# UPM-ROB-Lab/Vision-basedSensor

Measured on AMD Instinct MI355X. Metric: frames/sec (track->3D) at 1280x1024, 169 markers, higher is better.
Workload: dtype u8+f64; 1 GPU; BASELINE config 3/4: 4096 synthetic 1280x1024 gray uint8 frames per GPU (13x13 dots, seeded jitter+noise), resident in HBM; fused track->3D table + last-seen displacement; frames_per_gpu=4096, internal_batch=1536, pass_streams=2, markers=169, channels=1, world_size=1, backend=none (single process), distinct_devices=1, tracked_observations=692224, xyz_solved=692224, ncc_ambiguous_pixels=205, ncc_exact_pixels=11244250, ncc_counter_frames=839680

## Files before the change

include/vbs.h:

```cpp
#ifndef VBS_H
#define VBS_H

#include <stdint.h>

#ifdef __cplusplus
extern "C" {
#endif

#define VBS_OK          0
#define VBS_EINVAL     -1
#define VBS_ECAPACITY  -2
#define VBS_EHIP       -3
#define VBS_ENOMEM     -4
#define VBS_EINTERNAL  -5

#define VBS_DET_COLS    6
#define VBS_TABLE_COLS 10
#define VBS_FLAG_TRACKED 1
#define VBS_FLAG_XYZ     2
#define VBS_DISP_COLS   5
#define VBS_PLANE_COLS  5
#define VBS_DEVPLANE_COLS 9

typedef struct vbs_handle vbs_handle;
// ... 3 lines not shown
    float dist[5];
    float R[9];
    float T[3];
    float marker_diameter_mm;
} vbs_camera;

int vbs_create(int device, int height, int width, int max_markers, int max_batch, vbs_handle** out);
int vbs_destroy(vbs_handle* h);
const char* vbs_last_error(const vbs_handle* h);
int vbs_version(void);
#define VBS_OPT_GRAY_COEFFS      1
#define VBS_OPT_FORCE_SEQ_MATCH  2
#define VBS_OPT_NCC_MARGIN       4
#define VBS_OPT_STAGE_IMPL       5
#define VBS_OPT_BLUR_IMPL        6
#define VBS_OPT_PASS_STREAMS     7
#define VBS_OPT_LATENCY_FRAMES   8
int vbs_set_option(vbs_handle* h, int option, int value);
int vbs_mjpeg_probe(const uint8_t* jpeg, int64_t size, int32_t* info);
int vbs_mjpeg_entropy_batch(const uint8_t* buf, const int64_t* offs, const int32_t* sizes, int n, const int32_t* info,
                            uint32_t* ent, uint32_t* tab, int64_t* frame_base, int64_t* regions, uint16_t* qt, int32_t* status,
                            int threads);
int vbs_mjpeg_reconstruct(const uint32_t* ent, const uint32_t* tab, const int64_t* frame_base, const uint16_t* qt, int n,
                          const int32_t* info, uint8_t* planes, uint8_t* out, int64_t out_frame, int64_t out_row, void* stream);
#define VBS_MJPEG_SCAN_ALIGN      16
#define VBS_MJPEG_SCAN_GUARD      16
#define VBS_MJPEG_HUFF_SET_BYTES  8928
#define VBS_MJPEG_SUBSEQ_BITS     1024
#define VBS_MJPEG_DEVICE_BITS_MAX 2147418112
#define VBS_MJPEG_SHORT           1
int vbs_mjpeg_scan_batch(const uint8_t* buf, int64_t buf_size, const int64_t* offs, const int64_t* sizes, int n, const int32_t* info,
                         uint8_t* stage, int64_t stage_cap, int64_t* scan_off, int64_t* scan_bits, int32_t* table_set, void* sets,
                         int32_t* n_sets, int64_t* regions, uint16_t* qt, int32_t* status, int threads);
int vbs_mjpeg_huffman_device(const uint8_t* stage, const int64_t* scan_off, const int64_t* scan_bits, const int32_t* table_set,
                             const void* sets, int n_sets, int n, const int32_t* info, int subseq_bits, uint32_t* ent, uint32_t* tab,
                             int64_t* frame_base, int32_t* status, void* stream);
#define VBS_JPEG_BLOCK_BITS_MAX 1660
#define VBS_JPEG_HEADER_BYTES   623
int vbs_jpeg_encode_workspace(int width, int height, int n, int64_t* workspace_bytes, int64_t* payload_bytes,
                              int64_t* frame_bound);
int vbs_jpeg_encode(const uint8_t* frames, int n, int width, int height, int64_t stride_n, int64_t stride_row, int quality,
                    void* workspace, int64_t workspace_bytes, uint8_t* payload, int64_t payload_bytes, int64_t* offsets,
                    int32_t* sizes, void* stream);
int vbs_draw_tracking(const uint8_t* frames, int n, int height, int width, int64_t stride_n, int64_t stride_row,
                      const double* det, int max_markers, const float* table, const double* ref_xy, int m_ref,
                      int32_t* lastw, uint8_t* out, void* stream);
int vbs_contour_lut(uint8_t out[256]);
int vbs_step_lut(uint32_t out[256]);
int64_t vbs_format_csv(const int64_t* frameno, const int64_t* row, const int64_t* col, const double* const* fcols, int nf,
                       int64_t n, char* buf, int64_t cap, int threads);
int vbs_gaussian_taps_q8(int ksize, double sigma, int32_t* out);
int vbs_ncc_template(int l, double sigma, double* g, double* stats);
int vbs_ncc_trim_guard(int l, double sigma, int height, int width, double tbar_shift, double* min_d0);

int vbs_set_undistort(vbs_handle* h, const double* K9, const double* dist, int ndist, double* newK9, void* stream);
int vbs_undistort_frames(vbs_handle* h, const uint8_t* frames, int n, int channels, int64_t stride_n,
                         int64_t stride_row, uint8_t* out, void* stream);

int vbs_bgr2gray(vbs_handle* h, const uint8_t* frames, int n, int64_t stride_n, int64_t stride_row, uint8_t* gray,
                 void* stream);

int vbs_find_markers(vbs_handle* h, const uint8_t* frames, int n, int channels, int64_t stride_n,
                     int64_t stride_row, uint8_t* mask, uint8_t* area_mask, void* stream);

int vbs_ncc_map(vbs_handle* h, const uint8_t* frames, int n, int channels, int64_t stride_n,
                int64_t stride_row, double* ncc, void* stream);
int vbs_normxcorr2(vbs_handle* h, const uint8_t* area_mask, int n, double* ncc, uint8_t* mask,
                   void* stream);
int vbs_normxcorr2_general(int device, const double* tmpl, int th, int tw, const double* image, int h, int w, int mode,
                           double* out, void* stream);
int vbs_profile(vbs_handle* h, int enable);
int vbs_profile_read(vbs_handle* h, char* buf, int cap);
int vbs_frame_stats(vbs_handle* h, uint32_t* out, int n);
int vbs_stage_tables(vbs_handle* h, int n, uint32_t* ncomp, uint64_t* band_sums, uint32_t* area_first, int64_t* area_sums,
                     uint16_t* probe, uint32_t* slow);
int vbs_ellipse_table(vbs_handle* h, int n, double* out);
int vbs_ncc_counters(vbs_handle* h, uint64_t out[3], int reset);

int vbs_undistort_points(int device, const double* pts, int n, const vbs_camera* cam, double* out,
                         void* stream);
int vbs_calculate_3d(int device, const double* uvd, int n, const vbs_camera* cam, double* xyz,
                     int32_t* ok, void* stream);

#define VBS_PNP_SAMPLE            6
#define VBS_PNP_MAX_POINTS     1024
#define VBS_PNP_MAX_HYPOTHESES 4096
#define VBS_PNP_FEW_POINTS        1
#define VBS_PNP_NO_HYPOTHESIS     2
int vbs_pnp_ransac(int device, const double* world, int n_points, const double* image, const float* table,
                   const uint8_t* valid, int n_problems, const vbs_camera* cam, const int32_t* samples, int n_hyp,
                   double reproj_px, int32_t* hyp_count, double* hyp_pose, int32_t* status, double* pose,
                   int32_t* inlier_count, uint8_t* inlier_mask, double* errors, int32_t* winner, void* stream);

#define VBS_CALIB_MAX_VIEWS   64
#define VBS_CALIB_FEW_VIEWS    1
#define VBS_CALIB_DEGENERATE   2
int vbs_calibrate_camera(int device, const double* obj, int n_points, const double* img, int n_views, const uint8_t* view_mask,
                         int n_problems, int w, int h, int max_iter, double* homography, int32_t* view_void, int32_t* status,
                         double* K4, double* dist, double* R, double* T, double* rms, double* view_rms, double* std_intrinsics,
                         int32_t* iterations, void* stream);

int vbs_marker_center(vbs_handle* h, const uint8_t* mask, const uint8_t* area_mask, int n,
                      double* det, int32_t* counts, void* stream);

#define VBS_DIAM_COLS        24
#define VBS_DIAM_STATS_COLS   5
// ... 204 lines not shown
```

vision-basedsensor_amd/_lib.py:

```python
import ctypes as C
import os

_HERE = os.path.dirname(os.path.abspath(__file__))
LIB_PATH = os.path.join(_HERE, "csrc", "libvbs.so")

VBS_OK, VBS_EINVAL, VBS_ECAPACITY, VBS_EHIP, VBS_ENOMEM, VBS_EINTERNAL = 0, -1, -2, -3, -4, -5
DET_COLS, TABLE_COLS, DISP_COLS, PLANE_COLS, DEVPLANE_COLS = 6, 10, 5, 5, 9
FLAG_TRACKED, FLAG_XYZ = 1, 2
JPEG_BLOCK_BITS_MAX, JPEG_HEADER_BYTES = 1660, 623
MJPEG_SCAN_ALIGN, MJPEG_SCAN_GUARD, MJPEG_HUFF_SET_BYTES, MJPEG_SUBSEQ_BITS, MJPEG_SHORT = 16, 16, 8928, 1024, 1
SERIES_CHUNK, SERIES_REC_COLS, STATS_COLS, WINDOW_COLS = 32, 5, 5, 4
FIR_MAX_TAPS, FIR_TILE, AXIS_COLS, TOTAL_COLS = 255, 64, 4, 5
STEP_MAX_WINDOW, STEP_MAX_STEPS = 64, 64
POSE_COLS, POSEFIELD_COLS, POSE_GROUP = 8, 6, 8
FIELD_FRAMES, FIELD_MAX_SLOTS, FIELD_MAX_POINTS, PATCH_COLS, PATCH_GROUP = 4, 1024, 65536, 8, 8
PROJ_SLOTS, PROJ_CHUNK, PROJ_ROWS, PROJ_WG_SLOTS, PROJ_MAX_ROWS, PROJ_MAX_FRAMES, PROJ_MAX_SLOTS = 4, 64, 64, 16, 8192, 1048576, 1024
FIT_GROUP, PEAK_COLS = 4, 7
ENV_TILE, ENV_MAX_HALF = 64, 127
KIN_TILE, KIN_MAX_HALF, KIN_MAX_DEGREE = 64, 127, 3
MOM_CHUNK, MOM_WG_SLOTS, MOM_MAX_SLOTS = 32, 16, 1024
MODES_MAX, MODES_MAX_DIM, MODES_SWEEPS, MODES_MAX_ITERS, SCORE_GROUP = 16, 3072, 10, 4096, 8
STRAIN_COLS, LSTRAIN_COLS, MOTION_GROUP, LSTRAIN_GROUP, STRAIN_MAX_NBR = 16, 8, 8, 8, 12
ROBUST_MAX_HALF, ROBUST_TILE = 31, 64
DIAM_COLS, DIAM_STATS_COLS, DIAM_MAX_EXTENT = 24, 5, 512
PNP_SAMPLE, PNP_MAX_POINTS, PNP_MAX_HYPOTHESES, PNP_FEW_POINTS, PNP_NO_HYPOTHESIS = 6, 1024, 4096, 1, 2
CHESS_MAX_CANDIDATES, CHESS_MAX_PATTERN, CHESS_MAX_WIN = 256, 256, 15
CALIB_MAX_VIEWS, CALIB_FEW_VIEWS, CALIB_DEGENERATE = 64, 1, 2
IDS_MAX_MARKERS, IDS_MAX_LAYERS = 1024, 16
RETRACK_MAX, RETRACK_STATE_COLS, RETRACK_INFO_COLS = 1024, 6, 4
UNCERT_CAM, UNCERT_COV_COLS, UNCERT_DCOV_COLS, UNCERT_TOTAL_COLS, UNCERT_GROUP = 16, 7, 8, 8, 4
UNCERT_REF_COLS, UNCERT_WORK_COLS, NOISE_COLS = 55, 61, 10
POSECOV_COLS, POSECOV_GROUP = 17, 4
OPT_GRAY_COEFFS, OPT_FORCE_SEQ_MATCH, OPT_NCC_MARGIN, OPT_STAGE_IMPL, OPT_BLUR_IMPL, OPT_PASS_STREAMS, OPT_LATENCY_FRAMES = 1, 2, 4, 5, 6, 7, 8

SYMBOLS = ("vbs_create", "vbs_destroy", "vbs_last_error", "vbs_version", "vbs_contour_lut",
           "vbs_gaussian_taps_q8", "vbs_ncc_template", "vbs_ncc_trim_guard", "vbs_set_undistort", "vbs_undistort_frames", "vbs_find_markers", "vbs_ncc_map", "vbs_normxcorr2",
           "vbs_profile", "vbs_profile_read", "vbs_frame_stats", "vbs_undistort_points", "vbs_calculate_3d", "vbs_marker_center",
           "vbs_track", "vbs_solve3d", "vbs_track_to_3d", "vbs_displacement", "vbs_displacement_range", "vbs_displacement_f64",
           "vbs_plane_fit", "vbs_assign_ids", "vbs_set_option", "vbs_bgr2gray", "vbs_ncc_counters", "vbs_normxcorr2_general",
           "vbs_stage_tables", "vbs_ellipse_table", "vbs_deviation_plane", "vbs_format_csv", "vbs_mjpeg_probe", "vbs_mjpeg_entropy_batch",
           "vbs_mjpeg_reconstruct", "vbs_jpeg_encode_workspace", "vbs_jpeg_encode", "vbs_draw_tracking",
           "vbs_series_chunks", "vbs_series_stats", "vbs_series_stats_f64", "vbs_series_partial", "vbs_series_merge",
           "vbs_window_means", "vbs_displacement_from_frame", "vbs_mjpeg_scan_batch", "vbs_mjpeg_huffman_device",
           "vbs_step_lut", "vbs_threshold_bits", "vbs_measure_markers", "vbs_pnp_ransac",
           "vbs_chess_workspace", "vbs_chess_corners", "vbs_corner_subpix", "vbs_calibrate_camera",
           "vbs_retrack_workspace", "vbs_retrack",
           "vbs_uncert_points", "vbs_uncert_cov", "vbs_uncert_total", "vbs_pixel_noise", "vbs_pose_cov",
           "vbs_axis_displacement", "vbs_fir_series_f64",
           "vbs_step_response_f64", "vbs_find_steps_f64", "vbs_dwell_stats_f64", "vbs_pose_series",
           "vbs_field_map_f64", "vbs_patch_stats_f64", "vbs_project_series_f64", "vbs_harmonic_fit_f64", "vbs_window_moments_f64", "vbs_window_fit_f64",
           "vbs_poly_moments_f64", "vbs_poly_fit_f64",
           "vbs_motion_series_f64", "vbs_local_strain_f64", "vbs_hampel_series_f64",
           "vbs_cross_moments_f64", "vbs_covariance_f64", "vbs_leading_modes_f64", "vbs_mode_scores_f64")


class Camera(C.Structure):
    _fields_ = [("K", C.c_float * 9), ("dist", C.c_float * 5), ("R", C.c_float * 9),
                ("T", C.c_float * 3), ("marker_diameter_mm", C.c_float)]


class VbsError(RuntimeError):
    pass


def status_text(status: int, max_markers: int = 0) -> str:
    if status == VBS_ECAPACITY:
        return ("the frame exceeds the device workspace (more than 30720 runs in a mask, more than "
                f"{max_markers or 'max_markers'} band components, more than about 512 contours, or a contour thousands of rows "
                "long whose vertex moments would leave 64 bits)")
    if status == VBS_EINTERNAL:
        return ("a kernel's internal hand-shake timed out: the frame's result is not to be trusted (bounded wait expired; "
                "see VBS_EINTERNAL in include/vbs.h)")
    return "unexpected device status"


_lib = None


def lib():
    global _lib
    if _lib is not None:
        return _lib
    if not os.path.exists(LIB_PATH):
        raise VbsError(f"{LIB_PATH} is missing: build it with `python -c 'import __graft_entry__ as g; "
                       f"g.build()'` (hipcc, gfx950). There is no CPU fallback.")
    try:
        import torch
    except ImportError:
        pass
    L = C.CDLL(LIB_PATH)
    vp, i32, i64, f64 = C.c_void_p, C.c_int, C.c_int64, C.c_double
    cam_p = C.POINTER(Camera)
    sig = {
        "vbs_create": (i32, [i32, i32, i32, i32, i32, C.POINTER(vp)]),
        "vbs_destroy": (i32, [vp]),
        "vbs_last_error": (C.c_char_p, [vp]),
        "vbs_version": (i32, []),
        "vbs_contour_lut": (i32, [vp]),
        "vbs_gaussian_taps_q8": (i32, [i32, f64, vp]),
        "vbs_ncc_template": (i32, [i32, f64, vp, vp]),
        "vbs_ncc_trim_guard": (i32, [i32, f64, i32, i32, f64, vp]),
        "vbs_set_undistort": (i32, [vp, vp, vp, i32, vp, vp]),
        "vbs_undistort_frames": (i32, [vp, vp, i32, i32, i64, i64, vp, vp]),
        "vbs_find_markers": (i32, [vp, vp, i32, i32, i64, i64, vp, vp, vp]),
        "vbs_ncc_map": (i32, [vp, vp, i32, i32, i64, i64, vp, vp]),
        "vbs_normxcorr2": (i32, [vp, vp, i32, vp, vp, vp]),
        "vbs_profile": (i32, [vp, i32]),
        "vbs_profile_read": (i32, [vp, vp, i32]),
        "vbs_frame_stats": (i32, [vp, vp, i32]),
        "vbs_undistort_points": (i32, [i32, vp, i32, cam_p, vp, vp]),
        "vbs_calculate_3d": (i32, [i32, vp, i32, cam_p, vp, vp, vp]),
        "vbs_marker_center": (i32, [vp, vp, vp, i32, vp, vp, vp]),
        "vbs_track": (i32, [vp, vp, vp, i32, vp, i32, f64, vp, vp]),
        "vbs_solve3d": (i32, [vp, vp, i32, i32, cam_p, f64, vp]),
        "vbs_track_to_3d": (i32, [vp, vp, i32, i32, i64, i64, vp, i32, f64, cam_p, f64, vp, vp, vp, vp]),
        "vbs_displacement": (i32, [vp, vp, i32, i32, i32, f64, f64, vp, vp]),
        "vbs_displacement_range": (i32, [vp, vp, i32, i32, i32, f64, f64, i32, i32, vp, vp]),
        "vbs_displacement_f64": (i32, [i32, vp, i32, i32, i32, f64, f64, vp, vp]),
        "vbs_plane_fit": (i32, [vp, vp, i32, i32, vp, vp]),
        "vbs_assign_ids": (i32, [vp, vp, vp, i32, i32, vp, vp, i32, vp, vp]),
        "vbs_set_option": (i32, [vp, i32, i32]),
        "vbs_bgr2gray": (i32, [vp, vp, i32, i64, i64, vp, vp]),
        "vbs_ncc_counters": (i32, [vp, vp, i32]),
        "vbs_normxcorr2_general": (i32, [i32, vp, i32, i32, vp, i32, i32, i32, vp, vp]),
        "vbs_stage_tables": (i32, [vp, i32, vp, vp, vp, vp, vp, vp]),
        "vbs_ellipse_table": (i32, [vp, i32, vp]),
        "vbs_deviation_plane": (i32, [vp, vp, vp, vp, vp, vp, i32, i32, f64, vp, vp, vp]),
        "vbs_format_csv": (i64, [vp, vp, vp, vp, i32, i64, vp, i64, i32]),
        "vbs_mjpeg_probe": (i32, [vp, i64, vp]),
        "vbs_mjpeg_entropy_batch": (i32, [vp, vp, vp, i32, vp, vp, vp, vp, vp, vp, vp, i32]),
        "vbs_mjpeg_reconstruct": (i32, [vp, vp, vp, vp, i32, vp, vp, vp, i64, i64, vp]),
        "vbs_mjpeg_scan_batch": (i32, [vp, i64, vp, vp, i32, vp, vp, i64, vp, vp, vp, vp, vp, vp, vp, vp, i32]),
        "vbs_mjpeg_huffman_device": (i32, [vp, vp, vp, vp, vp, i32, i32, vp, i32, vp, vp, vp, vp, vp]),
        "vbs_jpeg_encode_workspace": (i32, [i32, i32, i32, vp, vp, vp]),
        "vbs_jpeg_encode": (i32, [vp, i32, i32, i32, i64, i64, i32, vp, i64, vp, i64, vp, vp, vp]),
        "vbs_draw_tracking": (i32, [vp, i32, i32, i32, i64, i64, vp, i32, vp, vp, i32, vp, vp, vp]),
        "vbs_series_chunks": (i32, [i32, i32]),
        "vbs_series_stats": (i32, [vp, vp, i32, i32, i32, vp, vp, vp]),
        "vbs_series_stats_f64": (i32, [i32, vp, i32, i32, i32, vp, vp, vp, vp]),
        "vbs_series_partial": (i32, [vp, vp, i32, i32, i32, vp, vp]),
        "vbs_series_merge": (i32, [vp, vp, i32, i32, vp, vp, vp]),
        "vbs_window_means": (i32, [vp, vp, i32, i32, vp, i32, vp, vp]),
        "vbs_displacement_from_frame": (i32, [vp, vp, i32, i32, i32, vp, vp]),
        "vbs_axis_displacement": (i32, [vp, vp, i32, i32, i32, vp, i32, i32, vp, vp, vp]),
        "vbs_fir_series_f64": (i32, [i32, vp, i32, i32, i32, i32, vp, i32, f64, i32, i32, vp, vp]),
        "vbs_step_response_f64": (i32, [i32, vp, i32, i32, i32, i32, i32, i32, vp, vp]),
        "vbs_find_steps_f64": (i32, [i32, vp, i32, i32, i32, i32, f64, i32, vp, vp]),
        "vbs_dwell_stats_f64": (i32, [i32, vp, i32, i32, i32, i32, vp, i32, i32, i32, vp, vp]),
        "vbs_pose_series": (i32, [vp, vp, i32, i32, i32, vp, vp, vp, i32, f64, f64, i32, i32, vp, vp, vp, vp]),
        "vbs_field_map_f64": (i32, [i32, vp, i32, i32, i32, i32, vp, vp, i32, f64, i32, i32, vp, vp]),
        "vbs_patch_stats_f64": (i32, [i32, vp, i32, i32, i32, vp, i32, f64, f64, vp, vp]),
        "vbs_project_series_f64": (i32, [i32, vp, i32, i32, i32, i32, vp, i32, vp, vp]),
        "vbs_harmonic_fit_f64": (i32, [i32, vp, i32, i32, i32, i32, i32, f64, vp, vp, vp]),
        "vbs_window_moments_f64": (i32, [i32, vp, i32, i32, i32, i32, vp, vp, i32, i32, i32, vp, vp]),
# ... 47 lines not shown
```

vision-basedsensor_amd/csrc/k_stage.hip:

```cpp
#include "stage_common.h"

#define ST_NT_SMALL 256
#define ST_NT 768

struct StageGeom {
    int H, W, WW, G, NB, R, maxm;
    u32 off_rec, off_bot, off_pq, off_mb, off_tmp;
    u32 mrec_cap, mrec_stride;
    u32 rec_cap, pq_cap, mom_comps;
    int stop;
    int retry;
};

template <int NT>
__device__ __forceinline__ u32 st_scan(u32 v, u32* tmp, u32* total) {
    const int lane = threadIdx.x & 63, wave = threadIdx.x >> 6;
    u32 inc = v;
#pragma unroll
    for (int d = 1; d < 64; d <<= 1) {
        const u32 t = __shfl_up(inc, d);
        if (lane >= d) inc += t;
    }
    if (lane == 63) tmp[wave] = inc;
    __syncthreads();
    if (wave == 0) {
        const u32 t = lane < NT / 64 ? tmp[lane] : 0u;
        u32 ti = t;
#pragma unroll
        for (int d = 1; d < NT / 64; d <<= 1) {
            const u32 o = __shfl_up(ti, d);
            if (lane >= d) ti += o;
        }
        if (lane < NT / 64) tmp[lane] = ti - t;
        if (lane == NT / 64 - 1) tmp[16] = ti;
    }
    __syncthreads();
    const u32 ex = inc - v + tmp[wave];
    *total = tmp[16];
    __syncthreads();
    return ex;
}

template <int NT>
__device__ __forceinline__ u32 seg_resolve(unsigned short* P, u32 sbase, u32 nseg, const unsigned short* rec_sid,
                                           const u32* rec_pos, u32 nrec, const u32* seg_pos, u32* comp_pos,
                                           unsigned short* cidmap, u32* tmp, u32 limit, const PairQ& Q) {
    const int tid = threadIdx.x;
    {
        const int np = min(*Q.n, Q.cap);
        for (int i = tid; i < np; i += NT) { const u32 pr = Q.q[i]; ccl_union(P, pr >> 16, pr & 0xFFFFu); }
    }
    __syncthreads();
    for (u32 i = 0; i < nseg; ++i) {
        u32 x = sbase + i, p;
        while ((p = ((volatile unsigned short*)P)[x]) != x) x = p;
        if (x != sbase + i) P[sbase + i] = (unsigned short)x;
    }
    __syncthreads();
    u32 nroot = 0;
    for (u32 i = 0; i < nseg; ++i) nroot += (P[sbase + i] == sbase + i);
    u32 ncomp;
    u32 c0 = st_scan<NT>(nroot, tmp, &ncomp);
    if (ncomp > limit) return NONE32;
    for (u32 i = 0; i < nseg; ++i)
        if (P[sbase + i] == sbase + i) { comp_pos[c0] = NONE32; P[sbase + i] = (unsigned short)(0x8000u | c0++); }
    __syncthreads();
    for (u32 i = 0; i < nseg; ++i) {
        const u32 v = P[sbase + i];
        if (!(v & 0x8000u)) P[sbase + i] = (unsigned short)(P[v] & 0x7FFFu);
    }
    __syncthreads();
    if (seg_pos) { for (u32 i = 0; i < nseg; ++i) atomicMin(&comp_pos[P[sbase + i] & 0x7FFFu], seg_pos[sbase + i]); }
    else { for (u32 r = tid; r < nrec; r += NT) atomicMin(&comp_pos[P[rec_sid[r]] & 0x7FFFu], rec_pos[r]); }
    __syncthreads();
    for (u32 c = tid; c < ncomp; c += NT) {
        const u32 p = comp_pos[c];
        u32 rank = 0;
        for (u32 q = 0; q < ncomp; ++q) rank += comp_pos[q] < p;
        cidmap[c] = (unsigned short)rank;
    }
    __syncthreads();
    return ncomp;
}

template <int NS, int NT>
__global__ __launch_bounds__(NT, 3) void k_stage(const u64* __restrict__ mask_all, const u64* __restrict__ area_all,
                                                    u32* __restrict__ ncomp_all, u64* __restrict__ band_sums,
                                                    u32* __restrict__ area_first, i64* __restrict__ area_sums,
                                                    unsigned short* __restrict__ probe_all, u32* __restrict__ fstat,
                                                    u32* __restrict__ slow_flag, u32* __restrict__ slow_total,
                                                    u32* __restrict__ mrec_all, StageGeom geo) {
    extern __shared__ __align__(16) unsigned char smem[];
    unsigned short* P = reinterpret_cast<unsigned short*>(smem);
    unsigned char* recb = smem + geo.off_rec;
    unsigned char* botb = smem + geo.off_bot;
    PairQ Q;
    Q.q = reinterpret_cast<u32*>(smem + geo.off_pq);
    Q.cap = (int)geo.pq_cap;
    u32* mb_cnt = reinterpret_cast<u32*>(smem + geo.off_mb);
    u32* mb_req = mb_cnt + NT;
    u32* tmp = reinterpret_cast<u32*>(smem + geo.off_tmp);
    int* misc = reinterpret_cast<int*>(tmp + 32);
    const int n = blockIdx.x, tid = threadIdx.x, lane = tid & 63, wave = tid >> 6;
    const int H = geo.H, W = geo.W, WW = geo.WW, G = geo.G, R = geo.R, maxm = geo.maxm;
    const int g = lane / WW, j = lane - g * WW;
    const bool act = g < G;
    const int blk = wave * G + g, y0 = blk * R;
    const bool hasl = j > 0, hasr = act && j + 1 < WW;
    const u64 vm = act ? valid_mask(j, W) : 0ull;
    const int NBW = geo.NB * WW, bj = act ? blk * WW + j : 0;
    const bool hasu = act && blk > 0;
    const u32 sbase = (u32)tid * SG_SEGMAX;
    Q.n = &misc[5];
    if (tid < 16) misc[tid] = 0;
    mb_cnt[tid] = 0;
    const int64_t fo = (int64_t)n * H * WW;
    const u32 rec_cap = geo.rec_cap;
    unsigned short* rec_sid = reinterpret_cast<unsigned short*>(recb);
    u32* rec_pos = reinterpret_cast<u32*>(recb + 2 * rec_cap);
    u32* rec_cnt = rec_pos + rec_cap;
    u32* rec_sx = rec_cnt + rec_cap;
    u32* rec_sy = rec_sx + rec_cap;
    u32* seg_pos = reinterpret_cast<u32*>(recb);
    u64* bot_mask = reinterpret_cast<u64*>(botb);
    unsigned short* bot_sid = reinterpret_cast<unsigned short*>(botb + (size_t)8 * SG_KB * NBW);
    u32* comp_pos = reinterpret_cast<u32*>(botb);
    unsigned short* cidmap = reinterpret_cast<unsigned short*>(botb + 4096);
    unsigned char* accb = botb + 4096 + 2048;
    auto hand_on = [&](u32 why) {
        if (tid == 0) { slow_flag[n] = why; atomicAdd(slow_total, 1u); }
    };
    if (geo.retry) {
        if (*slow_total == 0u) return;
        const u32 f = slow_flag[n];
        if (f != SLOW_SLOTS && f != SLOW_SEGS && f != SLOW_RECS && f != SLOW_PAIRS && f != SLOW_MAILBOX) return;
        __syncthreads();
        if (tid == 0) { slow_flag[n] = 0u; atomicSub(slow_total, 1u); }
    }
    __syncthreads();

    {
        constexpr int NA = NS / 2, NBL = NS / 2 - 1;
        const u64* M = mask_all + fo;
        auto ldraw = [&](int r) -> u64 {
            const int y = min(max(y0 + r, 0), H - 1);
            return M[(int64_t)y * WW + (act ? j : 0)];
        };
        auto rowval = [&](u64 raw, int r) -> u64 {
            const int y = y0 + r;
            return (act && y >= 0 && y < H) ? or_not(raw, vm) : ~0ull;
        };
        u64 pf[4];
#pragma unroll
        for (int i = 0; i < 4; ++i) pf[i] = ldraw(-NA + i);
        u64 cr[NBL + 1];
#pragma unroll
        for (int i = 0; i <= NBL; ++i) cr[i] = ~0ull;
        u64 h1 = ~0ull, a2[2] = {~0ull, ~0ull}, a4[4] = {~0ull, ~0ull, ~0ull, ~0ull};
        u64 a8[6] = {~0ull, ~0ull, ~0ull, ~0ull, ~0ull, ~0ull};
        u64 pm[SG_KB];
        u32 sid[SG_KB], cnt[SG_KB], sy[SG_KB], sk[SG_KB], pos[SG_KB];
#pragma unroll
        for (int k = 0; k < SG_KB; ++k) { pm[k] = 0; sid[k] = 0; cnt[k] = 0; sy[k] = 0; sk[k] = 0; pos[k] = 0; }
        u32 nseg = 0, la = NONE16, lb = NONE16, p63 = NONE16, prs0 = NONE16;
        bool fail = false;
        u64 firstB = 0;
        auto emit = [&](u32 sid_, u32 pos_, u32 cnt_, u32 sk_, u32 sy_) {
            const int r = atomicAdd(&misc[4], 1);
            if ((u32)r < rec_cap) {
                rec_sid[r] = (unsigned short)sid_; rec_pos[r] = pos_; rec_cnt[r] = cnt_;
                rec_sx[r] = 64u * (u32)j * cnt_ + sk_; rec_sy[r] = sy_;
            } else fail = true;
        };
        auto band_step = [&](const int q) __attribute__((always_inline)) {
            const int r = q - NA;
            const u64 v = rowval(pf[0], r);
            pf[0] = pf[1]; pf[1] = pf[2]; pf[2] = pf[3]; pf[3] = ldraw(r + 4);
#pragma unroll
            for (int i = NBL; i > 0; --i) cr[i] = cr[i - 1];
            cr[0] = v;
            const u64 n2 = h1 & v, n4 = a2[1] & n2;
            u64 e;
            if (NS == 14) {
                const u64 n8 = a4[3] & n4;
                e = a8[5] & n8;
                a8[5] = a8[4]; a8[4] = a8[3]; a8[3] = a8[2]; a8[2] = a8[1]; a8[1] = a8[0]; a8[0] = n8;
            } else {
                e = a4[3] & n4;
            }
            a4[3] = a4[2]; a4[2] = a4[1]; a4[1] = a4[0]; a4[0] = n4;
            a2[1] = a2[0]; a2[0] = n2;
            h1 = v;
            const int t = r - NBL;
            if (t < 0) return;
            const u64 eh = hwin<NS, true>(e, hasl, hasr);
            const u64 B = (act && y0 + t < H) ? and_not_and(cr[NBL], eh, vm) : 0ull;
            if (t == 0) firstB = B;
            bool live = false;
#pragma unroll
// ... 43 lines not shown
        for (int k = 0; k < SG_KB; ++k) {
            if (cnt[k]) emit(sid[k], pos[k], cnt[k], sk[k], sy[k]);
            if (act) { bot_mask[(size_t)k * NBW + bj] = pm[k]; bot_sid[(size_t)k * NBW + bj] = (unsigned short)sid[k]; }
        }
        if (fail) misc[6] = SLOW_SLOTS;
        __syncthreads();
        if (misc[6]) { hand_on((u32)misc[6]); return; }
        if (geo.stop == 2) return;
        if (hasu) {
            u64 N = firstB;
            u32 i = 0;
            while (N) {
                const u64 lowbit = N & (~N + 1ull), t2 = N + lowbit, gg = N & ~t2;
                N &= t2;
#pragma unroll
                for (int k = 0; k < SG_KB; ++k)
                    if (gg & bot_mask[(size_t)k * NBW + bj - WW]) pq_push(Q, sbase + i, bot_sid[(size_t)k * NBW + bj - WW]);
                ++i;
            }
        }
        __syncthreads();
        if (geo.stop == 3) return;
        const u32 nrec = (u32)misc[4];
        const u32 ncomp = seg_resolve<NT>(P, sbase, min(nseg, (u32)SG_SEGMAX), rec_sid, rec_pos, nrec, nullptr, comp_pos, cidmap, tmp,
                                      min((u32)maxm, 1024u), Q);
        if (misc[5] > Q.cap) { hand_on(SLOW_PAIRS); return; }
        if (ncomp == NONE32) { hand_on(SLOW_NCOMP); return; }
        if (geo.stop == 4) return;
        u32* acnt = reinterpret_cast<u32*>(accb);
        u64* asx = reinterpret_cast<u64*>(accb + 8 * ((maxm + 1) / 2));
        u64* asy = asx + maxm;
        for (u32 c = tid; c < ncomp; c += NT) { acnt[c] = 0; asx[c] = 0; asy[c] = 0; }
        __syncthreads();
        for (u32 r = tid; r < nrec; r += NT) {
            const u32 cid = cidmap[P[rec_sid[r]] & 0x7FFFu];
            atomicAdd(&acnt[cid], rec_cnt[r]); atomicAdd(&asx[cid], (u64)rec_sx[r]); atomicAdd(&asy[cid], (u64)rec_sy[r]);
        }
        __syncthreads();
        u64* bs = band_sums + (int64_t)n * maxm * 4;
        unsigned short* pr = probe_all + (int64_t)n * maxm * 4;
        for (u32 c = tid; c < ncomp; c += NT) {
            const u32 cn_ = acnt[c];
            const u64 sx = asx[c], sy_ = asy[c];
            bs[c * 4 + 0] = cn_; bs[c * 4 + 1] = sx; bs[c * 4 + 2] = sy_;
            const double cn = (double)cn_;
            const float xf = (float)((double)sx / cn), yf = (float)((double)sy_ / cn);
            const int ix = (int)floorf(xf), iy = (int)floorf(yf);
#pragma unroll
            for (int q = 0; q < 4; ++q) {
                const int px = ix + (q & 1), py = iy + (q >> 1);
                if (px < 0 || py < 0 || px >= W || py >= H) { pr[c * 4 + q] = (unsigned short)NONE16; continue; }
                const bool pair = (q & 1) == 0 && px + 1 < W && (px & 63) != 63;
                if ((q & 1) && px > 0 && (px & 63) != 0) continue;
                const int ob = py / R, oi = py - ob * R, ow = ob / G, og = ob - ow * G;
                const int owner = ow * 64 + og * WW + (px >> 6);
                const u32 slot = atomicAdd(&mb_cnt[owner], 1u);
                if (slot < ST_MB_CAP)
                    mb_req[owner * ST_MB_CAP + slot] = c | ((u32)q << 10) | ((u32)oi << 12) | ((u32)(px & 63) << 19) | ((u32)pair << 25);
                else misc[6] = SLOW_MAILBOX;
            }
        }
        if (tid == 0) { ncomp_all[n * 2 + 0] = ncomp; fstat[n * 8 + 5] = ncomp; misc[0] = 0; misc[4] = 0; misc[5] = 0; }
        __syncthreads();
        if (misc[6]) { hand_on((u32)misc[6]); return; }
        if (geo.stop == 10) return;
    }

    const u32 nband = ncomp_all[n * 2 + 0];
    u32 ncomp;
    u32* mrec = mrec_all + (size_t)n * geo.mrec_stride;
    unsigned short* pr = probe_all + (int64_t)n * maxm * 4;
    {
        const u64* A = area_all + fo;
        auto ldraw = [&](int r) -> u64 {
            const int y = min(max(y0 + r, 0), H - 1);
            return A[(int64_t)y * WW + (act ? j : 0)];
        };
        auto rowval = [&](u64 raw, int r) -> u64 {
            const int y = y0 + r;
            return (act && y >= 0 && y < H) ? or_not(raw, vm) : ~0ull;
        };
        u64 pf[4];
#pragma unroll
        for (int i = 0; i < 4; ++i) pf[i] = ldraw(-5 + i);
        u64 e5[4] = {~0ull, ~0ull, ~0ull, ~0ull}, d5[4] = {0, 0, 0, 0};
        u64 o1 = 0, o2 = 0;
        u32 l1 = 0, l2 = 0, r1 = 0, r2 = 0;
        u64 rowm[2] = {0, 0};
        const u32 nreq = min(mb_cnt[tid], (u32)ST_MB_CAP);
        for (u32 q = 0; q < nreq; ++q) {
            const u32 rr = (mb_req[tid * ST_MB_CAP + q] >> 12) & 127u;
            if (rr < 64) rowm[0] |= 1ull << rr; else rowm[1] |= 1ull << (rr - 64);
        }
        auto row_asked = [&](int c) -> bool { return ((c < 64 ? rowm[0] >> c : rowm[1] >> (c - 64)) & 1ull) != 0; };
        u64 pm[SG_KO];
        u32 sid[SG_KO];
        int mo[SG_KO][NMOM];
#pragma unroll
        for (int k = 0; k < SG_KO; ++k) {
            pm[k] = 0; sid[k] = 0;
#pragma unroll
            for (int q = 0; q < NMOM; ++q) mo[k][q] = 0;
        }
        u32 nseg = 0, la = NONE16, lb = NONE16, p63 = NONE16, prs0 = NONE16;
        u32 why = 0;
        u64 firstB = 0;
        int e4 = 0;
        const int tch = R >> 1;
        const int mthr = R <= 64 ? 900 : 56;
        auto emit_mom = [&](u32 sid_, int (&m)[NMOM]) {
            const int r = atomicAdd(&misc[7], 1);
            if ((u32)r < geo.mrec_cap) {
                uint4* dst = reinterpret_cast<uint4*>(mrec + (size_t)r * 16);
                dst[0] = make_uint4(sid_, (u32)m[0], (u32)m[1], (u32)m[2]);
                dst[1] = make_uint4((u32)m[3], (u32)m[4], (u32)m[5], (u32)m[6]);
                dst[2] = make_uint4((u32)m[7], (u32)m[8], (u32)m[9], (u32)m[10]);
                dst[3] = make_uint4((u32)m[11], (u32)m[12], (u32)m[13], (u32)m[14]);
            } else why = SLOW_RECS;
#pragma unroll
            for (int q = 0; q < NMOM; ++q) m[q] = 0;
        };
        auto open_step = [&](const int q) __attribute__((always_inline)) {
            const int r = q - 5;
            const u64 v = rowval(pf[0], r);
            pf[0] = pf[1]; pf[1] = pf[2]; pf[2] = pf[3]; pf[3] = ldraw(r + 4);
            u64 ve = v & e5[0] & e5[1] & e5[2] & e5[3];
            e5[3] = e5[2]; e5[2] = e5[1]; e5[1] = e5[0]; e5[0] = v;
            u64 er = 0;
            if (r >= -1) {
                const int ye = y0 + r - 2;
                er = hwin<5, true>(ve, hasl, hasr);
                er = (act && ye >= 0 && ye < H) ? (er & vm) : 0ull;
            }
            const u64 vd = er | d5[0] | d5[1] | d5[2] | d5[3];
            d5[3] = d5[2]; d5[2] = d5[1]; d5[1] = d5[0]; d5[0] = er;
            const int rho = r - 4;
            if (rho < -1) return;
            u64 o0 = hwin<5, false>(vd, hasl, hasr);
            {
                const int y = y0 + rho;
                o0 = (act && y >= 0 && y < H) ? (o0 & vm) : 0ull;
            }
            u32 l0 = dpp_shr1((u32)(o0 >> 63)), r0 = dpp_shl1((u32)o0 & 1u);
            if (!hasl) l0 = 0;
            if (!hasr) r0 = 0;
            const int c = rho - 1;
            bool live = false;
#pragma unroll
            for (int k = 0; k < SG_KO; ++k) live |= pm[k] != 0ull;
            if (c >= 0) {
                const bool top = (y0 + c) == 0;
#pragma unroll
                for (int qq = 0; qq < 2; ++qq) {
                    if (qq == 1 && !top) continue;
                    const u64 a = qq ? 0ull : o1, bq = qq ? o1 : o0;
                    const u32 an = qq ? 0u : r1, bn = qq ? r1 : r0;
                    if (a | bq | an | bn) {
                        e4 += euler_quads(a, bq, an, bn);
                        if (j == 0) e4 += (int)((a ^ bq) & 1ull);
                    }
                }
            }
            if (c >= 0 && __any(o1 != 0ull || live || row_asked(c))) {
                const u64 B = o1;
                if (c == 0) firstB = B;
                const u64 rB = brev64(B);
                u64 Rn[SG_KO];
                const u64 claimed = seg_update<SG_KO, true, true>(B, rB, pm, sid, Rn, Q);
#pragma unroll
                for (int k = 0; k < SG_KO; ++k) pm[k] = Rn[k];
                u64 N = B & ~claimed;
                while (N) {
                    const u64 lowbit = N & (~N + 1ull), t2 = N + lowbit, gg = N & ~t2;
                    N &= t2;
                    bool done = false;
#pragma unroll
                    for (int k = 0; k < SG_KO; ++k) {
                        if (!done && pm[k] == 0ull) {
                            if (mo[k][0]) emit_mom(sid[k], mo[k]);
                            if (nseg < SG_SEGMAX) {
                                sid[k] = sbase + nseg; P[sbase + nseg] = (unsigned short)(sbase + nseg);
                                seg_pos[sbase + nseg] = (u32)(y0 + c) * (u32)W + 64u * (u32)j + (u32)(__ffsll((long long)gg) - 1);
                            } else why = SLOW_SEGS;
                            ++nseg;
                            pm[k] = gg;
                            done = true;
                        }
                    }
                    if (!done) why = SLOW_SLOTS;
                }
                if (__any(((B >> 63) | B) & 1ull)) seg_hlinks<SG_KO, true>(pm, sid, hasr, p63, prs0, la, lb, Q);
                else { p63 = NONE16; prs0 = NONE16; }
                if (row_asked(c)) {
                    for (u32 qq = 0; qq < nreq; ++qq) {
                        const u32 rq = mb_req[tid * ST_MB_CAP + qq];
                        if (((rq >> 12) & 127u) != (u32)c) continue;
                        const u32 q0 = (rq >> 10) & 3u;
                        for (u32 d = 0; d <= ((rq >> 25) & 1u); ++d) {
                            const u32 kb = ((rq >> 19) & 63u) + d;
                            u32 s = NONE16;
#pragma unroll
                            for (int k = 0; k < SG_KO; ++k)
                                if ((pm[k] >> kb) & 1ull) s = sid[k];
                            pr[(rq & 1023u) * 4 + q0 + d] = (unsigned short)s;
// ... 55 lines not shown
        if (geo.stop == 12) return;
        if (hasu && firstB) {
            u64 N = firstB;
            u32 i = 0;
            while (N) {
                const u64 lowbit = N & (~N + 1ull), t2 = N + lowbit, gg = N & ~t2;
                N &= t2;
                const u64 ga = gg | (gg << 1) | (gg >> 1);
#pragma unroll
                for (int k = 0; k < SG_KO; ++k) {
                    if (ga & bot_mask[(size_t)k * NBW + bj - WW]) pq_push(Q, sbase + i, bot_sid[(size_t)k * NBW + bj - WW]);
                    if ((gg & 1ull) && hasl && (bot_mask[(size_t)k * NBW + bj - WW - 1] >> 63))
                        pq_push(Q, sbase + i, bot_sid[(size_t)k * NBW + bj - WW - 1]);
                    if ((gg >> 63) && hasr && (bot_mask[(size_t)k * NBW + bj - WW + 1] & 1ull))
                        pq_push(Q, sbase + i, bot_sid[(size_t)k * NBW + bj - WW + 1]);
                }
                ++i;
            }
        }
        __syncthreads();
        if (geo.stop == 13) return;
        ncomp = seg_resolve<NT>(P, sbase, min(nseg, (u32)SG_SEGMAX), nullptr, nullptr, 0, seg_pos, comp_pos, cidmap, tmp,
                            min((u32)maxm, (u32)CCL_OPEN_COMPS), Q);
        if (misc[5] > Q.cap) { hand_on(16u + SLOW_PAIRS); return; }
        if (ncomp == NONE32) { hand_on(16u + SLOW_NCOMP); return; }
        if ((int)ncomp - misc[0] / 4 != 0) {
            hand_on(16u + SLOW_HOLES);
            return;
        }
    }
    if (geo.stop == 14) return;
    u32* anchor = reinterpret_cast<u32*>(accb);
    u64* acc = reinterpret_cast<u64*>(accb + 4 * CCL_OPEN_COMPS);
    {
        u32* first = area_first + (int64_t)n * maxm;
        for (u32 c = tid; c < ncomp; c += NT) {
            const u32 pos = comp_pos[c], cid = cidmap[c], py = pos / (u32)W;
            anchor[cid] = (py << 16) | (pos - py * (u32)W);
            first[cid] = pos;
        }
    }
    i64* as = area_sums + (int64_t)n * maxm * VBS_AREA_SUMS;
    const u32 nmrec = (u32)misc[7];
    for (u32 c0 = 0; c0 < ncomp; c0 += geo.mom_comps) {
        const u32 nc = min(geo.mom_comps, ncomp - c0);
        for (u32 c = tid; c < nc * NMOM; c += NT) acc[c] = 0;
        __syncthreads();
        for (u32 r = tid; r < nmrec; r += NT) {
            const uint4* src = reinterpret_cast<const uint4*>(mrec + (size_t)r * 16);
            const uint4 w0 = src[0], w1 = src[1], w2 = src[2], w3 = src[3];
            const u32 s = w0.x, cid = (u32)cidmap[P[s] & 0x7FFFu] - c0;
            if (cid >= nc) continue;
            const u32 ot = s / SG_SEGMAX, ol = ot & 63u, og = ol / (u32)WW;
            const int ox = 64 * (int)(ol - og * (u32)WW) + 32, oy = (int)((ot >> 6) * (u32)G + og) * R + (R >> 1);
            const u32 fp = anchor[cid + c0];
            const i64 m[NMOM] = {(int)w0.y, (int)w0.z, (int)w0.w, (int)w1.x, (int)w1.y, (int)w1.z, (int)w1.w, (int)w2.x,
                                 (int)w2.y, (int)w2.z, (int)w2.w, (int)w3.x, (int)w3.y, (int)w3.z, (int)w3.w};
            i64 o[NMOM];
            shift_moments_i64(m, (i64)(ox - (int)(fp & 0xFFFFu)), (i64)(oy - (int)(fp >> 16)), o);
            u64* a = acc + cid * NMOM;
#pragma unroll
            for (int q = 0; q < NMOM; ++q)
                if (o[q]) atomicAdd(&a[q], (u64)o[q]);
        }
        __syncthreads();
        for (u32 c = tid; c < nc * NMOM; c += NT) as[(c0 + c / NMOM) * VBS_AREA_SUMS + (c % NMOM)] = (i64)acc[c];
        __syncthreads();
    }
    for (u32 e = tid; e < nband * 4; e += NT) {
        const u32 v = pr[e];
        if (v != NONE16) pr[e] = cidmap[P[v] & 0x7FFFu];
    }
    if (tid == 0) { ncomp_all[n * 2 + 1] = ncomp; fstat[n * 8 + 6] = ncomp; fstat[n * 8 + 4] = 0; }
}

int stage_threads(const vbs_handle* h, int nb) {
    if (h->stage_impl == 3) return ST_NT;
    const int G = 64 / h->WW, R768 = (h->H + (ST_NT / 64) * G - 1) / ((ST_NT / 64) * G);
    if (h->bp.ns == 8) return R768 <= 8 ? ST_NT_SMALL : ST_NT;
    return (h->stage_impl == 4 || nb >= 512) ? ST_NT_SMALL : ST_NT;
}

static bool stage_geom(const vbs_handle* h, const Workspace& w, StageGeom* g, size_t* lds_bytes, int nt) {
    if (h->W > 4096 || h->H > 2048 || h->maxm > 1024) return false;
    const int G = 64 / h->WW, NB = (nt / 64) * G;
    const int R = (h->H + NB - 1) / NB;
    if (R > 128 || R < 1) return false;
    g->H = h->H; g->W = h->W; g->WW = h->WW; g->G = G; g->NB = NB; g->R = R; g->maxm = h->maxm;
    g->stop = VBS_KNOB("VBS_STAGE_STOP");
    g->retry = 0;
    const size_t NBW = (size_t)NB * h->WW;
    auto up16 = [](size_t x) { return (x + 15) / 16 * 16; };
    const bool half = nt < ST_NT;
    g->rec_cap = (u32)(half ? 768 : SG_REC);
    g->pq_cap = (u32)(half ? 1536 : SG_PQ);
    g->mom_comps = (u32)(half ? CCL_MOM_COMPS / 4 : CCL_MOM_COMPS);
    const size_t par = up16((size_t)nt * SG_SEGMAX * 2);
    size_t rec = up16((size_t)g->rec_cap * 18);
    if (rec < (size_t)nt * SG_SEGMAX * 4) rec = (size_t)nt * SG_SEGMAX * 4;
    const size_t bot = up16((size_t)SG_KB * NBW * 10);
    const size_t acc_band = up16((size_t)(8 * ((h->maxm + 1) / 2)) + 16 * (size_t)h->maxm);
    const size_t acc_open = up16((size_t)4 * CCL_OPEN_COMPS + (size_t)g->mom_comps * NMOM * 8);
    const size_t comp = 4096 + 2048 + (acc_band > acc_open ? acc_band : acc_open);
    const size_t botc = bot > comp ? bot : comp;
    const size_t pq = (size_t)g->pq_cap * 4, mb = (size_t)nt * 4 * (1 + ST_MB_CAP), misc = 32 * 4 + 16 * 4;
    g->off_rec = (u32)par;
    g->off_bot = (u32)(par + rec);
    g->off_pq = (u32)(par + rec + botc);
    g->off_mb = (u32)(g->off_pq + pq);
    g->off_tmp = (u32)(g->off_mb + mb);
    *lds_bytes = g->off_tmp + misc;
    g->mrec_stride = w.stage_mrec ? 16u * (u32)SG_REC : 2u * (u32)h->H * (u32)h->WW;
    g->mrec_cap = g->mrec_stride / 16u < (u32)SG_REC ? g->mrec_stride / 16u : (u32)SG_REC;
    return *lds_bytes <= (size_t)(half ? 160 * 1024 / 3 - 256 : 160 * 1024);
}

template <int NS, int NT>
static bool stage_launch_t(vbs_handle* h, Workspace& w, int nb, const StageGeom& g, size_t lds, hipStream_t s) {
    size_t& set = h->stage_lds_set[NT == ST_NT ? 0 : 1];
    if (lds > set) {
        if (hipFuncSetAttribute(reinterpret_cast<const void*>(k_stage<NS, NT>), hipFuncAttributeMaxDynamicSharedMemorySize,
                                (int)lds) != hipSuccess) {
            (void)hipGetLastError();
            return false;
        }
        set = lds;
    }
    VBS_LAUNCH(h, s, g.retry ? "k_stage_retry" : "k_stage", (k_stage<NS, NT>), dim3(nb), dim3(NT), lds, s, w.mask_bits, w.area_bits, w.ncomp,
               w.band_sums, w.area_first, w.area_sums, w.probe, w.fstat, w.slow_flag, w.slow_total,
               w.stage_mrec ? w.stage_mrec : w.wbase, g);
    return true;
}

bool launch_stage(vbs_handle* h, Workspace& w, int nb, int nt, hipStream_t s) {
    StageGeom g;
    size_t lds = 0;
    if (nt < ST_NT && stage_geom(h, w, &g, &lds, ST_NT_SMALL) &&
        (h->bp.ns == 14 ? stage_launch_t<14, ST_NT_SMALL>(h, w, nb, g, lds, s) : stage_launch_t<8, ST_NT_SMALL>(h, w, nb, g, lds, s))) {
        if (stage_geom(h, w, &g, &lds, ST_NT)) {
            g.retry = 1;
            (void)(h->bp.ns == 14 ? stage_launch_t<14, ST_NT>(h, w, nb, g, lds, s) : stage_launch_t<8, ST_NT>(h, w, nb, g, lds, s));
        }
        return true;
    }
    if (!stage_geom(h, w, &g, &lds, ST_NT)) return false;
    return h->bp.ns == 14 ? stage_launch_t<14, ST_NT>(h, w, nb, g, lds, s) : stage_launch_t<8, ST_NT>(h, w, nb, g, lds, s);
}
```

vision-basedsensor_amd/csrc/stage_common.h:

```cpp
#pragma once
#include "ccl_common.h"

#define ST_MB_CAP 8
#define SG_KB 4
#define SG_KO 3
#define SG_SEGMAX 8
#define SG_PQ 4096
#define NONE32 0xFFFFFFFFu
#define SLOW_SLOTS 1
#define SLOW_NCOMP 2
#define SLOW_MAILBOX 3
#define SLOW_HOLES 4
#define SLOW_VERTEX 5
#define SLOW_SEGS 6
#define SLOW_RECS 7
#define SLOW_PAIRS 8


__device__ __forceinline__ u64 mk64(u32 lo, u32 hi) { return ((u64)hi << 32) | lo; }
__device__ __forceinline__ u64 brev64(u64 x) {
    return mk64(__builtin_bitreverse32((u32)(x >> 32)), __builtin_bitreverse32((u32)x));
}

__device__ __forceinline__ u64 and_not_and(u64 a, u64 b, u64 c) {
    return mk64((u32)a & ~(u32)b & (u32)c, (u32)(a >> 32) & ~(u32)(b >> 32) & (u32)(c >> 32));
}
__device__ __forceinline__ u64 or_not(u64 a, u64 b) { return mk64((u32)a | ~(u32)b, (u32)(a >> 32) | ~(u32)(b >> 32)); }

__device__ __forceinline__ u64 shift_from_right(u64 x, int s, bool hasr, u32 fill) {
    const u32 lo = (u32)x, hi = (u32)(x >> 32);
    u32 rlo = dpp_shl1(lo);
    if (!hasr) rlo = fill;
    return mk64(__builtin_amdgcn_alignbit(hi, lo, (u32)s), __builtin_amdgcn_alignbit(rlo, hi, (u32)s));
}
__device__ __forceinline__ u64 shift_from_left(u64 x, int s, bool hasl, u32 fill) {
    const u32 lo = (u32)x, hi = (u32)(x >> 32);
    u32 lhi = dpp_shr1(hi);
    if (!hasl) lhi = fill;
    return mk64(__builtin_amdgcn_alignbit(lo, lhi, (u32)(32 - s)), __builtin_amdgcn_alignbit(hi, lo, (u32)(32 - s)));
}

template <int N, bool ERODE>
__device__ __forceinline__ u64 hwin(u64 v, bool hasl, bool hasr) {
    const u32 fill = ERODE ? ~0u : 0u;
    constexpr int NL = N / 2 + 1, NR = N - N / 2;
    u64 f = v, b = v;
    int have = 1;
#pragma unroll
    for (int it = 0; it < 5; ++it) {
        if (have >= NR) break;
        const int s = have < NR - have ? have : NR - have;
        const u64 t = shift_from_right(f, s, hasr, fill);
        f = ERODE ? (f & t) : (f | t);
        have += s;
    }
    have = 1;
#pragma unroll
    for (int it = 0; it < 5; ++it) {
        if (have >= NL) break;
        const int s = have < NL - have ? have : NL - have;
        const u64 t = shift_from_left(b, s, hasl, fill);
        b = ERODE ? (b & t) : (b | t);
        have += s;
    }
    return ERODE ? (f & b) : (f | b);
}

__device__ __forceinline__ u64 fill_runs(u64 B, u64 rB, u64 S) {
    const u64 su = S + B;
// ... 143 lines not shown
```

Measured before the change: 314,900 frames/s.

## Shrink stage kernel work to per-frame marker bounding box

Adds a prepass in the stage kernel that scans the mask and area bitmaps to find the occupied x/y bounding box of each frame. It then recomputes the block geometry (word columns, groups, rows per block) so threads cover only the box plus a guard, shortening the per-thread row count. The box also changes LDS sizing of the bottom buffers, and requests outside the box are dropped. The cost is an extra full read of both bitmaps plus atomics and a sync, and the savings depend on markers occupying only part of the frame.

```diff
diff --git a/include/vbs.h b/include/vbs.h
--- a/include/vbs.h
+++ b/include/vbs.h
@@ -79,6 +79,7 @@
 int vbs_gaussian_taps_q8(int ksize, double sigma, int32_t* out);
 int vbs_ncc_template(int l, double sigma, double* g, double* stats);
 int vbs_ncc_trim_guard(int l, double sigma, int height, int width, double tbar_shift, double* min_d0);
+int vbs_stage_box_geom(int height, int width, int ns, int threads, int xlo, int xhi, int ylo, int yhi, int* out);
 
 int vbs_set_undistort(vbs_handle* h, const double* K9, const double* dist, int ndist, double* newK9, void* stream);
 int vbs_undistort_frames(vbs_handle* h, const uint8_t* frames, int n, int channels, int64_t stride_n,
diff --git a/vision-basedsensor_amd/_lib.py b/vision-basedsensor_amd/_lib.py
--- a/vision-basedsensor_amd/_lib.py
+++ b/vision-basedsensor_amd/_lib.py
@@ -34,7 +34,7 @@
 OPT_GRAY_COEFFS, OPT_FORCE_SEQ_MATCH, OPT_NCC_MARGIN, OPT_STAGE_IMPL, OPT_BLUR_IMPL, OPT_PASS_STREAMS, OPT_LATENCY_FRAMES = 1, 2, 4, 5, 6, 7, 8
 
 SYMBOLS = ("vbs_create", "vbs_destroy", "vbs_last_error", "vbs_version", "vbs_contour_lut",
-           "vbs_gaussian_taps_q8", "vbs_ncc_template", "vbs_ncc_trim_guard", "vbs_set_undistort", "vbs_undistort_frames", "vbs_find_markers", "vbs_ncc_map", "vbs_normxcorr2",
+           "vbs_gaussian_taps_q8", "vbs_ncc_template", "vbs_ncc_trim_guard", "vbs_stage_box_geom", "vbs_set_undistort", "vbs_undistort_frames", "vbs_find_markers", "vbs_ncc_map", "vbs_normxcorr2",
            "vbs_profile", "vbs_profile_read", "vbs_frame_stats", "vbs_undistort_points", "vbs_calculate_3d", "vbs_marker_center",
            "vbs_track", "vbs_solve3d", "vbs_track_to_3d", "vbs_displacement", "vbs_displacement_range", "vbs_displacement_f64",
            "vbs_plane_fit", "vbs_assign_ids", "vbs_set_option", "vbs_bgr2gray", "vbs_ncc_counters", "vbs_normxcorr2_general",
@@ -100,6 +100,7 @@
         "vbs_gaussian_taps_q8": (i32, [i32, f64, vp]),
         "vbs_ncc_template": (i32, [i32, f64, vp, vp]),
         "vbs_ncc_trim_guard": (i32, [i32, f64, i32, i32, f64, vp]),
+        "vbs_stage_box_geom": (i32, [i32, i32, i32, i32, i32, i32, i32, i32, vp]),
         "vbs_set_undistort": (i32, [vp, vp, vp, i32, vp, vp]),
         "vbs_undistort_frames": (i32, [vp, vp, i32, i32, i64, i64, vp, vp]),
         "vbs_find_markers": (i32, [vp, vp, i32, i32, i64, i64, vp, vp, vp]),
diff --git a/vision-basedsensor_amd/csrc/k_stage.hip b/vision-basedsensor_amd/csrc/k_stage.hip
--- a/vision-basedsensor_amd/csrc/k_stage.hip
+++ b/vision-basedsensor_amd/csrc/k_stage.hip
@@ -10,6 +10,7 @@
     u32 rec_cap, pq_cap, mom_comps;
     int stop;
     int retry;
+    int bbox;
 };
 
 template <int NT>
@@ -102,19 +103,12 @@
     u32* tmp = reinterpret_cast<u32*>(smem + geo.off_tmp);
     int* misc = reinterpret_cast<int*>(tmp + 32);
     const int n = blockIdx.x, tid = threadIdx.x, lane = tid & 63, wave = tid >> 6;
-    const int H = geo.H, W = geo.W, WW = geo.WW, G = geo.G, R = geo.R, maxm = geo.maxm;
-    const int g = lane / WW, j = lane - g * WW;
-    const bool act = g < G;
-    const int blk = wave * G + g, y0 = blk * R;
-    const bool hasl = j > 0, hasr = act && j + 1 < WW;
-    const u64 vm = act ? valid_mask(j, W) : 0ull;
-    const int NBW = geo.NB * WW, bj = act ? blk * WW + j : 0;
-    const bool hasu = act && blk > 0;
+    const int H = geo.H, W = geo.W, WWF = geo.WW, maxm = geo.maxm;
     const u32 sbase = (u32)tid * SG_SEGMAX;
     Q.n = &misc[5];
-    if (tid < 16) misc[tid] = 0;
+    if (tid < 16) misc[tid] = (tid == 8 || tid == 10) ? 0x7FFFFFFF : (tid == 9 || tid == 11) ? -1 : 0;
     mb_cnt[tid] = 0;
-    const int64_t fo = (int64_t)n * H * WW;
+    const int64_t fo = (int64_t)n * H * WWF;
     const u32 rec_cap = geo.rec_cap;
     unsigned short* rec_sid = reinterpret_cast<unsigned short*>(recb);
     u32* rec_pos = reinterpret_cast<u32*>(recb + 2 * rec_cap);
@@ -123,7 +117,6 @@
     u32* rec_sy = rec_sx + rec_cap;
     u32* seg_pos = reinterpret_cast<u32*>(recb);
     u64* bot_mask = reinterpret_cast<u64*>(botb);
-    unsigned short* bot_sid = reinterpret_cast<unsigned short*>(botb + (size_t)8 * SG_KB * NBW);
     u32* comp_pos = reinterpret_cast<u32*>(botb);
     unsigned short* cidmap = reinterpret_cast<unsigned short*>(botb + 4096);
     unsigned char* accb = botb + 4096 + 2048;
@@ -137,14 +130,62 @@
         __syncthreads();
         if (tid == 0) { slow_flag[n] = 0u; atomicSub(slow_total, 1u); }
     }
-    __syncthreads();
+    StageBox tb = {0, WWF, geo.G, geo.NB, geo.R, 0};
+    u64 sacc = 0;
+    int sfirst = 0x7FFFFFFF, slast = -1, sj = 0;
+    if (geo.bbox) {
+        const int g0 = lane / WWF;
+        sj = lane - g0 * WWF;
+        const int yb = (wave * geo.G + g0) * geo.R, ylast = min(yb + geo.R - 1, H - 1);
+        const u64* Mp = mask_all + fo + sj;
+        const u64* Ap = area_all + fo + sj;
+#pragma unroll 1
+        for (int r = 0; r < geo.R; r += 8) {
+            u64 m[8], a[8];
+#pragma unroll
+            for (int i = 0; i < 8; ++i) {
+                const int64_t o = (int64_t)min(yb + r + i, ylast) * WWF;
+                m[i] = Mp[o]; a[i] = Ap[o];
+            }
+#pragma unroll
+            for (int i = 0; i < 8; ++i) {
+                const u64 v = m[i] | a[i];
+                const int y = min(yb + r + i, ylast);
+                sacc |= v;
+                if (v) { sfirst = min(sfirst, y); slast = max(slast, y); }
+            }
+        }
+        if (g0 >= geo.G) sacc = 0;
+    }
+    __syncthreads();
+    if (geo.bbox) {
+        if (sacc) {
+            atomicMin(&misc[8], 64 * sj + __ffsll((long long)sacc) - 1);
+            atomicMax(&misc[9], 64 * sj + 63 - __clzll((long long)sacc));
+            atomicMin(&misc[10], sfirst);
+            atomicMax(&misc[11], slast);
+        }
+        __syncthreads();
+        const int xlo = __builtin_amdgcn_readfirstlane(misc[8]), xhi = __builtin_amdgcn_readfirstlane(misc[9]);
+        const int ylo = __builtin_amdgcn_readfirstlane(misc[10]), yhi = __builtin_amdgcn_readfirstlane(misc[11]);
+        tb = stage_box_geom(W, WWF, geo.G, geo.NB, geo.R, NT, NS / 2, xlo, xhi, ylo, yhi);
+    }
+    const int WW = tb.WW, G = tb.G, NB = tb.NB, R = tb.R, ja = tb.ja, ylo = tb.ylo;
+    const int g = lane / WW, jl = lane - g * WW, j = ja + jl;
+    const bool act = g < G;
+    const int blk = wave * G + g, y0 = ylo + blk * R;
+    const bool hasl = jl > 0, hasr = act && jl + 1 < WW;
+    const u64 vm = act ? valid_mask(j, W) : 0ull;
+    const int NBW = NB * WW, bj = act ? blk * WW + jl : 0;
+    const bool hasu = act && blk > 0;
+    unsigned short* bot_sid = reinterpret_cast<unsigned short*>(botb + (size_t)8 * SG_KB * NBW);
 
     {
         constexpr int NA = NS / 2, NBL = NS / 2 - 1;
         const u64* M = mask_all + fo;
         auto ldraw = [&](int r) -> u64 {
             const int y = min(max(y0 + r, 0), H - 1);
-            return M[(int64_t)y * WW + (act ? j : 0)];
+            return M[(int64_t)y * WWF + (act ? j : 0)];
         };
         auto rowval = [&](u64 raw, int r) -> u64 {
             const int y = y0 + r;
@@ -294,8 +335,14 @@
                 if (px < 0 || py < 0 || px >= W || py >= H) { pr[c * 4 + q] = (unsigned short)NONE16; continue; }
                 const bool pair = (q & 1) == 0 && px + 1 < W && (px & 63) != 63;
                 if ((q & 1) && px > 0 && (px & 63) != 0) continue;
-                const int ob = py / R, oi = py - ob * R, ow = ob / G, og = ob - ow * G;
-                const int owner = ow * 64 + og * WW + (px >> 6);
+                const int ry = py - ylo, wj = (px >> 6) - ja;
+                if (ry < 0 || ry >= NB * R || wj < 0 || wj >= WW) {
+                    pr[c * 4 + q] = (unsigned short)NONE16;
+                    if (pair) pr[c * 4 + q + 1] = (unsigned short)NONE16;
+                    continue;
+                }
+                const int ob = ry / R, oi = ry - ob * R, ow = ob / G, og = ob - ow * G;
+                const int owner = ow * 64 + og * WW + wj;
                 const u32 slot = atomicAdd(&mb_cnt[owner], 1u);
                 if (slot < ST_MB_CAP)
                     mb_req[owner * ST_MB_CAP + slot] = c | ((u32)q << 10) | ((u32)oi << 12) | ((u32)(px & 63) << 19) | ((u32)pair << 25);
@@ -316,7 +363,7 @@
         const u64* A = area_all + fo;
         auto ldraw = [&](int r) -> u64 {
             const int y = min(max(y0 + r, 0), H - 1);
-            return A[(int64_t)y * WW + (act ? j : 0)];
+            return A[(int64_t)y * WWF + (act ? j : 0)];
         };
         auto rowval = [&](u64 raw, int r) -> u64 {
             const int y = y0 + r;
@@ -391,7 +438,7 @@
 #pragma unroll
             for (int k = 0; k < SG_KO; ++k) live |= pm[k] != 0ull;
             if (c >= 0) {
-                const bool top = (y0 + c) == 0;
+                const bool top = (y0 + c) == ylo;
 #pragma unroll
                 for (int qq = 0; qq < 2; ++qq) {
                     if (qq == 1 && !top) continue;
@@ -553,7 +600,7 @@
             const u32 s = w0.x, cid = (u32)cidmap[P[s] & 0x7FFFu] - c0;
             if (cid >= nc) continue;
             const u32 ot = s / SG_SEGMAX, ol = ot & 63u, og = ol / (u32)WW;
-            const int ox = 64 * (int)(ol - og * (u32)WW) + 32, oy = (int)((ot >> 6) * (u32)G + og) * R + (R >> 1);
+            const int ox = 64 * (ja + (int)(ol - og * (u32)WW)) + 32, oy = ylo + (int)((ot >> 6) * (u32)G + og) * R + (R >> 1);
             const u32 fp = anchor[cid + c0];
             const i64 m[NMOM] = {(int)w0.y, (int)w0.z, (int)w0.w, (int)w1.x, (int)w1.y, (int)w1.z, (int)w1.w, (int)w2.x,
                                  (int)w2.y, (int)w2.z, (int)w2.w, (int)w3.x, (int)w3.y, (int)w3.z, (int)w3.w};
@@ -603,8 +650,11 @@
     const size_t acc_band = up16((size_t)(8 * ((h->maxm + 1) / 2)) + 16 * (size_t)h->maxm);
     const size_t acc_open = up16((size_t)4 * CCL_OPEN_COMPS + (size_t)g->mom_comps * NMOM * 8);
     const size_t comp = 4096 + 2048 + (acc_band > acc_open ? acc_band : acc_open);
-    const size_t botc = bot > comp ? bot : comp;
     const size_t pq = (size_t)g->pq_cap * 4, mb = (size_t)nt * 4 * (1 + ST_MB_CAP), misc = 32 * 4 + 16 * 4;
+    const size_t limit = (size_t)(half ? 160 * 1024 / 3 - 256 : 160 * 1024);
+    const size_t botn = up16((size_t)SG_KB * nt * 10);
+    g->bbox = h->bp.ns == 14 && !VBS_KNOB("VBS_STAGE_BBOX_OFF") && par + rec + (botn > comp ? botn : comp) + pq + mb + misc <= limit;
+    const size_t botu = g->bbox ? botn : bot, botc = botu > comp ? botu : comp;
     g->off_rec = (u32)par;
     g->off_bot = (u32)(par + rec);
     g->off_pq = (u32)(par + rec + botc);
@@ -613,7 +663,19 @@
     *lds_bytes = g->off_tmp + misc;
     g->mrec_stride = w.stage_mrec ? 16u * (u32)SG_REC : 2u * (u32)h->H * (u32)h->WW;
     g->mrec_cap = g->mrec_stride / 16u < (u32)SG_REC ? g->mrec_stride / 16u : (u32)SG_REC;
-    return *lds_bytes <= (size_t)(half ? 160 * 1024 / 3 - 256 : 160 * 1024);
+    return *lds_bytes <= limit;
+}
+
+extern "C" int vbs_stage_box_geom(int height, int width, int ns, int threads, int xlo, int xhi, int ylo, int yhi, int* out) {
+    if (!out || height < 1 || width < 1 || (ns != 14 && ns != 8) || (threads != ST_NT && threads != ST_NT_SMALL)) return VBS_EINVAL;
+    const int WW = (width + 63) / 64;
+    if (WW > 64 || width > 4096 || height > 2048) return VBS_EINVAL;
+    const int G = 64 / WW, NB = (threads / 64) * G, R = (height + NB - 1) / NB;
+    if (R > 128) return VBS_EINVAL;
+    const StageBox b = stage_box_geom(width, WW, G, NB, R, threads, ns / 2, xlo, xhi, ylo, yhi);
+    const int v[12] = {WW, G, NB, R, b.ja, b.WW, b.G, b.NB, b.R, b.ylo, ns / 2, b.R != R};
+    for (int i = 0; i < 12; ++i) out[i] = v[i];
+    return VBS_OK;
 }
 
 template <int NS, int NT>
@@ -640,6 +702,7 @@
         (h->bp.ns == 14 ? stage_launch_t<14, ST_NT_SMALL>(h, w, nb, g, lds, s) : stage_launch_t<8, ST_NT_SMALL>(h, w, nb, g, lds, s))) {
         if (stage_geom(h, w, &g, &lds, ST_NT)) {
             g.retry = 1;
+            g.bbox = 0;
             (void)(h->bp.ns == 14 ? stage_launch_t<14, ST_NT>(h, w, nb, g, lds, s) : stage_launch_t<8, ST_NT>(h, w, nb, g, lds, s));
         }
         return true;
diff --git a/vision-basedsensor_amd/csrc/stage_common.h b/vision-basedsensor_amd/csrc/stage_common.h
--- a/vision-basedsensor_amd/csrc/stage_common.h
+++ b/vision-basedsensor_amd/csrc/stage_common.h
@@ -15,6 +15,21 @@
 #define SLOW_SEGS 6
 #define SLOW_RECS 7
 #define SLOW_PAIRS 8
+
+struct StageBox { int ja, WW, G, NB, R, ylo; };
+__host__ __device__ inline StageBox stage_box_geom(int W, int WW, int G, int NB, int R, int nt, int guard, int xlo, int xhi, int ylo,
+                                                   int yhi) {
+    const StageBox full = {0, WW, G, NB, R, 0};
+    if (xlo > xhi || ylo > yhi) return full;
+    const int xa = xlo - guard > 0 ? xlo - guard : 0, xb = xhi + guard < W - 1 ? xhi + guard : W - 1;
+    const int ja = xa >> 6, WWe = (xb >> 6) - ja + 1;
+    const int Ge = 64 / WWe, NBe = (nt / 64) * Ge, Rmin = (R + 1) >> 1;
+    int Re = (yhi - ylo + NBe) / NBe;
+    if (Re < Rmin) Re = Rmin;
+    if (Re >= R) return full;
+    const StageBox box = {ja, WWe, Ge, NBe, Re, ylo};
+    return box;
+}
 
 
 __device__ __forceinline__ u64 mk64(u32 lo, u32 hi) { return ((u64)hi << 32) | lo; }
```

Measured after the change: 327,600 frames/s (median of 6 runs). 4.0% higher.
